# jeffreyyu0602/quantized-training

Measured on AMD Instinct MI355X. Metric: quantized_elements_per_sec, higher is better.
Workload: dtype bf16; 1 GPU; llama-2-7b-shaped LLaMA (32 layers, hidden 4096, random init) WikiText-style window eval B=1 S=1024 stride 512, fake-quant activation=e4m3 weight=e4m3, --quantize_forward gemm (weights re-quantized every forward); route=eager, parallelism=dp1 (windows round-robin, metric all_gather only), launch=hipGraph replay, valid=True

## Files before the change

### quantized-training_amd/csrc/qt_model_ops.hip

```cpp
#include <hip/hip_runtime.h>
#include <stdint.h>

#include "../../include/qt_hip.h"
#include "qt_device.h"
#include "qt_dispatch.h"
#include "qt_formats.h"
#include "qt_value_codes.h"
#include "qt_value_rows.h"

namespace {

constexpr int kNormThreads = 256;
constexpr int kNormMaxVec = 8;

struct NormExtra {
    uint2 *y8[2];
    qt_format fmt[2];
    int e5m2[2];
};

template <int FQ, bool ADD = false, int EXTRA = 0, int NV = kNormMaxVec>
__global__ __launch_bounds__(kNormThreads) void rmsnorm_kernel(const uint4 *__restrict__ x, const uint4 *__restrict__ w,
                                                               uint4 *__restrict__ y, int nvec, float inv_cols, float eps,
                                                               uint2 *__restrict__ y8, qt_format fmt,
// ... 123 lines not shown
        y[i] = uint4{o[0], o[1], o[2], o[3]};
    }
}

template <bool E5M2>
__global__ __launch_bounds__(256) void silu_mul_fq8_kernel(const uint4 *__restrict__ g, const uint4 *__restrict__ u,
                                                           uint4 *__restrict__ y, uint2 *__restrict__ y8, size_t nvec,
                                                           qt_format fmt, size_t cv, size_t rs_g, size_t rs_u) {
    for (size_t i = (size_t)blockIdx.x * 256 + threadIdx.x; i < nvec; i += (size_t)gridDim.x * 256) {
        const size_t row = i / cv, col = i - row * cv;
        const uint4 a = g[row * rs_g + col], b = u[row * rs_u + col];
        const uint32_t p[4] = {a.x, a.y, a.z, a.w}, q[4] = {b.x, b.y, b.z, b.w};
        uint32_t o[4];
#pragma unroll
        for (int j = 0; j < 4; ++j) {
            const float g0 = bf_lo(p[j]), g1 = bf_hi(p[j]);
            const float s0 = bf16_round(g0 / (1.0f + expf(-g0))), s1 = bf16_round(g1 / (1.0f + expf(-g1)));
            o[j] = pack_bf16x2(s0 * bf_lo(q[j]), s1 * bf_hi(q[j]));
        }
        const uint2 codes = fq8_hw_vec8<E5M2>(o, fmt);
        y[i] = uint4{o[0], o[1], o[2], o[3]};
        y8[i] = codes;
    }
}

struct RopeArgs {
    const uint16_t *x;
    uint16_t *y;
    const uint16_t *cos, *sin;
    long B, S, H, D;
    size_t nvec;
    long rsv;
};

__device__ __forceinline__ void rope_one(const RopeArgs &a, size_t i) {
    const long dv = a.D / 8;
    const long d8 = (long)(i % dv);
    const size_t bsh = i / dv;
    const size_t bs = bsh / (size_t)a.H;
    const long half = dv / 2;
    const bool low = d8 < half;
    const size_t in_row = bs * (size_t)a.rsv + (bsh % (size_t)a.H) * dv;
    const uint4 xv = *(const uint4 *)(a.x + (in_row + d8) * 8);
    const uint4 pv = *(const uint4 *)(a.x + (in_row + (low ? d8 + half : d8 - half)) * 8);
    const uint4 cv = *(const uint4 *)(a.cos + (bs * dv + d8) * 8);
    const uint4 sv = *(const uint4 *)(a.sin + (bs * dv + d8) * 8);
    const uint32_t X[4] = {xv.x, xv.y, xv.z, xv.w}, P[4] = {pv.x, pv.y, pv.z, pv.w};
    const uint32_t C[4] = {cv.x, cv.y, cv.z, cv.w}, S[4] = {sv.x, sv.y, sv.z, sv.w};
    const float sgn = low ? -1.0f : 1.0f;
    uint32_t o[4];
#pragma unroll
    for (int j = 0; j < 4; ++j) {
        const float a0 = bf16_round(bf_lo(X[j]) * bf_lo(C[j])), a1 = bf16_round(bf_hi(X[j]) * bf_hi(C[j]));
        const float b0 = bf16_round(sgn * bf_lo(P[j]) * bf_lo(S[j])), b1 = bf16_round(sgn * bf_hi(P[j]) * bf_hi(S[j]));
        o[j] = pack_bf16x2(a0 + b0, a1 + b1);
    }
    *(uint4 *)(a.y + i * 8) = uint4{o[0], o[1], o[2], o[3]};
}

__global__ __launch_bounds__(256) void rope_kernel(RopeArgs q, RopeArgs k) {
    const size_t total = q.nvec + k.nvec;
    for (size_t i = (size_t)blockIdx.x * 256 + threadIdx.x; i < total; i += (size_t)gridDim.x * 256) {
        if (i < q.nvec) rope_one(q, i);
        else rope_one(k, i - q.nvec);
    }
}

struct RopeFqArgs {
    RopeArgs r;
    qt_format fmt;
    uint8_t *y8;
    int e5m2;
    int inner;
    qt_format inner_fmt;
    const uint16_t *map;
    const uint16_t *rows_lds;
};

template <bool CODES = false>
__device__ __forceinline__ void rope_fq_token(const RopeFqArgs &a, size_t bs0, uint32_t tpb, size_t tokens) {
    const uint32_t dv = (uint32_t)a.r.D / 8, half = dv / 2, nv = (uint32_t)a.r.H * dv;
    const uint32_t S = (uint32_t)a.r.S;
    for (uint32_t i = threadIdx.x; i < tpb * nv; i += 256) {
        const uint32_t lt = tpb == 1 ? 0u : i / nv, v = i - lt * nv;
        const size_t bs = bs0 + lt;
        if (bs >= tokens) break;
        const uint32_t b = (uint32_t)(bs / S), s = (uint32_t)(bs - (size_t)b * S);
        const uint16_t *xrow = a.r.x + bs * (size_t)a.r.rsv * 8;
        const uint16_t *crow = a.r.cos + bs * dv * 8, *srow = a.r.sin + bs * dv * 8;
        const uint32_t h = v / dv, d8 = v - h * dv;
        const bool low = d8 < half;
        const uint4 xv = *(const uint4 *)(xrow + (size_t)v * 8);
        uint32_t out[4] = {xv.x, xv.y, xv.z, xv.w};
        if (a.r.cos) {
            const uint4 pv = *(const uint4 *)(xrow + (size_t)(low ? v + half : v - half) * 8);
            const uint4 cv = *(const uint4 *)(crow + d8 * 8);
            const uint4 sv = *(const uint4 *)(srow + d8 * 8);
            const uint32_t X[4] = {xv.x, xv.y, xv.z, xv.w}, P[4] = {pv.x, pv.y, pv.z, pv.w};
            const uint32_t C[4] = {cv.x, cv.y, cv.z, cv.w}, S[4] = {sv.x, sv.y, sv.z, sv.w};
            const float sgn = low ? -1.0f : 1.0f;
#pragma unroll
            for (int j = 0; j < 4; ++j) {
                float a0 = bf16_round(bf_lo(X[j]) * bf_lo(C[j])), a1 = bf16_round(bf_hi(X[j]) * bf_hi(C[j]));
                if (!CODES && a.inner) {
                    if (a.map) {
                        const Rounder<kFmtRows> rin{a.fmt, a.rows_lds, a.map};
                        a0 = qt_u2f(rin(qt_f2u(a0)));
                        a1 = qt_u2f(rin(qt_f2u(a1)));
                    } else {
                        a0 = qt_u2f(qt_fp_sat_u32(qt_f2u(a0), a.inner_fmt.p0, a.inner_fmt.p1, a.inner_fmt.fhi));
                        a1 = qt_u2f(qt_fp_sat_u32(qt_f2u(a1), a.inner_fmt.p0, a.inner_fmt.p1, a.inner_fmt.fhi));
                    }
                }
                const float b0 = bf16_round(sgn * bf_lo(P[j]) * bf_lo(S[j])), b1 = bf16_round(sgn * bf_hi(P[j]) * bf_hi(S[j]));
                out[j] = pack_bf16x2(a0 + b0, a1 + b1);
            }
        }
        const size_t o = (((size_t)b * (size_t)a.r.H + h) * (size_t)a.r.S + s) * dv + d8;
        if (CODES || a.y8) {
            const uint2 codes = a.e5m2 ? fq8_hw_vec8<true>(out, a.fmt) : fq8_hw_vec8<false>(out, a.fmt);
            *(uint2 *)(a.y8 + o * 8) = codes;
        } else if (a.map) {
            const Rounder<kFmtRows> rnd{a.fmt, a.rows_lds, a.map};
            const uint32_t oin[4] = {out[0], out[1], out[2], out[3]};
            fq_rows_words<4, false>(oin, out, rnd);
        } else {
#pragma unroll
            for (int j = 0; j < 4; ++j) {
                const uint32_t r0 = qt_fp_sat_u32(out[j] << 16, a.fmt.p0, a.fmt.p1, a.fmt.fhi);
                const uint32_t r1 = qt_fp_sat_u32(out[j] & 0xFFFF0000u, a.fmt.p0, a.fmt.p1, a.fmt.fhi);
                out[j] = (r0 >> 16) | (r1 & 0xFFFF0000u);
            }
        }
        if (a.r.y) *(uint4 *)(a.r.y + o * 8) = uint4{out[0], out[1], out[2], out[3]};
    }
}

__global__ __launch_bounds__(256) void rope_fq_kernel(RopeFqArgs q, RopeFqArgs k, unsigned tpb) {
    __shared__ uint4 s_rope_rows[512];
    if (q.map) {
        const uint4 *gr = (const uint4 *)(q.map + QT_MAP_ENTRIES);
        const int nrows = (q.fmt.p1 & 2) ? 512 : 256;
        for (int i = threadIdx.x; i < nrows; i += 256) s_rope_rows[i] = gr[i];
        __syncthreads();
        q.rows_lds = k.rows_lds = (const uint16_t *)s_rope_rows;
    }
    const size_t tokens = (size_t)q.r.B * (size_t)q.r.S;
    for (size_t bs = (size_t)blockIdx.x * tpb; bs < tokens; bs += (size_t)gridDim.x * tpb) {
        rope_fq_token(q, bs, tpb, tokens);
        rope_fq_token(k, bs, tpb, tokens);
    }
}

struct ValueArgs {
    const uint16_t *v;
    uint8_t *vt8;
    long sb, sh, sk, Sk;
    int H, nkb;
    qt_format fmt;
};

template <bool VE5M2, int VD, bool CODES = false>
__global__ __launch_bounds__(256) void rope_fq_value_kernel(RopeFqArgs q, RopeFqArgs k, ValueArgs v, unsigned rope_blocks, unsigned tpb) {
    __shared__ __attribute__((aligned(16))) uint8_t tile[VD * 128];
    if (blockIdx.x < rope_blocks) {
        const size_t tokens = (size_t)q.r.B * (size_t)q.r.S;
        for (size_t bs = (size_t)blockIdx.x * tpb; bs < tokens; bs += (size_t)rope_blocks * tpb) {
            rope_fq_token<CODES>(q, bs, tpb, tokens);
            rope_fq_token<CODES>(k, bs, tpb, tokens);
        }
    } else {
        const unsigned vb = blockIdx.x - rope_blocks;
        value_codes_block<VE5M2, VD>(tile, v.v, v.vt8, (int)(vb % (unsigned)v.nkb), (long)(vb / (unsigned)v.nkb), v.H, v.Sk, v.sb, v.sh, v.sk, v.fmt);
    }
}

struct ValueRowsArgs {
    const uint16_t *v;
    uint16_t *vt;
    long sb, sh, sk, Sk;
    int H, nkb;
};
struct WeightPassArgs {
    const uint4 *w;
    uint4 *wq;
    size_t nvec;
    unsigned blocks;
};

__global__ __launch_bounds__(256) void rope_map_value_kernel(RopeFqArgs q, RopeFqArgs k, ValueRowsArgs v, WeightPassArgs wp, unsigned rope_blocks,
                                                             unsigned tpb) {
    __shared__ __attribute__((aligned(16))) uint16_t tile[value_rows_tile_elems<64>()];
    __shared__ uint4 s_rows[512];
    {
        const uint4 *gr = (const uint4 *)(q.map + QT_MAP_ENTRIES);
        const int nrows = (q.fmt.p1 & 2) ? 512 : 256;
        for (int i = threadIdx.x; i < nrows; i += 256) s_rows[i] = gr[i];
        __syncthreads();
        q.rows_lds = k.rows_lds = (const uint16_t *)s_rows;
    }
    if (blockIdx.x < wp.blocks) {
        const Rounder<kFmtRows> rnd{q.fmt, (const uint16_t *)s_rows, q.map};
        constexpr int kU = 4;
        const size_t stride = (size_t)wp.blocks * 256;
        for (size_t i0 = (size_t)blockIdx.x * 256 + threadIdx.x; i0 < wp.nvec; i0 += stride * kU) {
            uint4 a[kU];
#pragma unroll
            for (int u = 0; u < kU; ++u)
                if (i0 + u * stride < wp.nvec) a[u] = wp.w[i0 + u * stride];
#pragma unroll
            for (int u = 0; u < kU; ++u) {
                if (i0 + u * stride < wp.nvec) {
                    const uint32_t in[4] = {a[u].x, a[u].y, a[u].z, a[u].w};
                    uint32_t o[4];
                    fq_rows_words<4, false>(in, o, rnd);
                    wp.wq[i0 + u * stride] = uint4{o[0], o[1], o[2], o[3]};
                }
            }
        }
        return;
    }
    const unsigned bid = blockIdx.x - wp.blocks;
    if (bid < rope_blocks) {
        const size_t tokens = (size_t)q.r.B * (size_t)q.r.S;
        for (size_t bs = (size_t)bid * tpb; bs < tokens; bs += (size_t)rope_blocks * tpb) {
            rope_fq_token(q, bs, tpb, tokens);
            rope_fq_token(k, bs, tpb, tokens);
        }
    } else {
        const unsigned vb = bid - rope_blocks;
        const Rounder<kFmtRows> rnd{q.fmt, (const uint16_t *)s_rows, q.map};
        value_t_rows_block<64>(tile, rnd, v.v, v.vt, v.H, v.Sk, v.sb, v.sh, v.sk, (long)(vb / (unsigned)v.nkb), (int)(vb % (unsigned)v.nkb), (int)threadIdx.x);
    }
}

struct LnArgs {
    const uint4 *x, *res, *w, *b;
    uint4 *y, *yq;
    uint2 *y8;
    long rows;
    int nvec;
    float inv_cols, eps;
    qt_format fmt;
    int n_extra;
    NormExtra extra;
};

template <int G, int FQ, bool ADD, int NV = kNormMaxVec>
__global__ __launch_bounds__(256) void layernorm_kernel(LnArgs a) {
    constexpr int RPB = 256 / G;
    __shared__ float s_part[2][4];
    const int sub = threadIdx.x / G, lane = threadIdx.x % G;
    const long row = (long)blockIdx.x * RPB + sub;
    if (G == 64 && row >= a.rows) return;
    const size_t base = (size_t)row * (size_t)a.nvec;
    uint4 v[NV];
    float sum = 0.0f;
#pragma unroll
    for (int i = 0; i < NV; ++i) {
        const int c = lane + i * G;
        if (c < a.nvec) {
            v[i] = a.x[base + c];
            if constexpr (ADD) {
                const uint4 r = a.res[base + c];
                v[i].x = pack_bf16x2(bf_lo(v[i].x) + bf_lo(r.x), bf_hi(v[i].x) + bf_hi(r.x));
                v[i].y = pack_bf16x2(bf_lo(v[i].y) + bf_lo(r.y), bf_hi(v[i].y) + bf_hi(r.y));
                v[i].z = pack_bf16x2(bf_lo(v[i].z) + bf_lo(r.z), bf_hi(v[i].z) + bf_hi(r.z));
                v[i].w = pack_bf16x2(bf_lo(v[i].w) + bf_lo(r.w), bf_hi(v[i].w) + bf_hi(r.w));
            }
            sum += (bf_lo(v[i].x) + bf_hi(v[i].x)) + (bf_lo(v[i].y) + bf_hi(v[i].y)) + (bf_lo(v[i].z) + bf_hi(v[i].z)) +
                   (bf_lo(v[i].w) + bf_hi(v[i].w));
        }
    }
    auto reduce = [&](float t, int slot) {
#pragma unroll
        for (int off = 32; off >= 1; off >>= 1) t += __shfl_xor(t, off, 64);
        if constexpr (G == 256) {
            if ((threadIdx.x & 63) == 0) s_part[slot][threadIdx.x >> 6] = t;
            __syncthreads();
            t = (s_part[slot][0] + s_part[slot][1]) + (s_part[slot][2] + s_part[slot][3]);
        }
        return t;
    };
    const float mean = reduce(sum, 0) * a.inv_cols;
    float sq = 0.0f;
#pragma unroll
    for (int i = 0; i < NV; ++i) {
        const int c = lane + i * G;
        if (c < a.nvec) {
            const uint32_t q[4] = {v[i].x, v[i].y, v[i].z, v[i].w};
#pragma unroll
            for (int j = 0; j < 4; ++j) {
                const float d0 = bf_lo(q[j]) - mean, d1 = bf_hi(q[j]) - mean;
                sq += d0 * d0;
                sq += d1 * d1;
            }
        }
    }
    const float rstd = rsqrtf(reduce(sq, 1) * a.inv_cols + a.eps);
#pragma unroll
    for (int i = 0; i < NV; ++i) {
        const int c = lane + i * G;
        if (c < a.nvec) {
            const uint4 ww = a.w[c], bb = a.b[c];
            const uint32_t q[4] = {v[i].x, v[i].y, v[i].z, v[i].w}, g[4] = {ww.x, ww.y, ww.z, ww.w}, h[4] = {bb.x, bb.y, bb.z, bb.w};
            uint32_t o[4];
#pragma unroll
            for (int j = 0; j < 4; ++j)
                o[j] = pack_bf16x2(bf_lo(g[j]) * (rstd * (bf_lo(q[j]) - mean)) + bf_lo(h[j]),
                                   bf_hi(g[j]) * (rstd * (bf_hi(q[j]) - mean)) + bf_hi(h[j]));
            a.y[base + c] = uint4{o[0], o[1], o[2], o[3]};
            if constexpr (FQ != 0) {
                for (int e = 0; e < a.n_extra; ++e) {
                    uint32_t t[4] = {o[0], o[1], o[2], o[3]};
                    a.extra.y8[e][base + c] = a.extra.e5m2[e] ? fq8_hw_vec8<true>(t, a.extra.fmt[e]) : fq8_hw_vec8<false>(t, a.extra.fmt[e]);
                }
                const uint2 codes = fq8_hw_vec8<FQ == 2>(o, a.fmt);
                if (a.yq) a.yq[base + c] = uint4{o[0], o[1], o[2], o[3]};
                a.y8[base + c] = codes;
            }
        }
    }
// ... 263 lines not shown
static int launch_layernorm_any(const LnArgs &a, int fq, bool with_residual, void *stream);

int qt_layernorm_bf16(const uint16_t *x, const uint16_t *residual, const uint16_t *weight, const uint16_t *bias, uint16_t *y,
                      uint16_t *yq, uint8_t *y8, long rows, long cols, float eps, const qt_format *fmt, void *stream) {
    if (rows * cols == 0) return QT_OK;
    if (!x || !weight || !bias || !y || rows < 0 || cols < 0 || (yq && !y8)) return QT_ERR_BAD_ARG;
    const int fq = y8 ? qt_fp8_code(fmt) : 0;
    if (y8 && !fq) return QT_ERR_BAD_ARG;
    if (cols % 8 || cols > (long)kNormThreads * kNormMaxVec * 8 ||
        (((uintptr_t)x | (uintptr_t)residual | (uintptr_t)weight | (uintptr_t)bias | (uintptr_t)y | (uintptr_t)yq) & 15u) || ((uintptr_t)y8 & 7u))
        return QT_ERR_UNALIGNED;
    LnArgs a{(const uint4 *)x, (const uint4 *)residual, (const uint4 *)weight, (const uint4 *)bias, (uint4 *)y, (uint4 *)yq, (uint2 *)y8,
             rows, (int)(cols / 8), 1.0f / (float)cols, eps, fmt && fq ? *fmt : qt_format{}, 0, NormExtra{}};
    return launch_layernorm_any(a, fq, residual != nullptr, stream);
}

int qt_layernorm_consumers_bf16(const uint16_t *x, const uint16_t *residual, const uint16_t *weight, const uint16_t *bias, uint16_t *y,
                                uint16_t *yq, long rows, long cols, float eps, int consumers, uint8_t *const *y8,
                                const qt_format *const *fmt, void *stream) {
    if (rows * cols == 0) return QT_OK;
    if (!x || !weight || !bias || !y || rows < 0 || cols < 0 || consumers < 2 || consumers > 3 || !y8 || !fmt) return QT_ERR_BAD_ARG;
    int code[3] = {0, 0, 0};
    for (int i = 0; i < consumers; ++i) {
        if (!y8[i] || !fmt[i] || ((uintptr_t)y8[i] & 7u)) return QT_ERR_BAD_ARG;
        code[i] = qt_fp8_code(fmt[i]);
        if (!code[i]) return QT_ERR_BAD_ARG;
    }
    if (cols % 8 || cols > (long)kNormThreads * kNormMaxVec * 8 ||
        (((uintptr_t)x | (uintptr_t)residual | (uintptr_t)weight | (uintptr_t)bias | (uintptr_t)y | (uintptr_t)yq) & 15u))
        return QT_ERR_UNALIGNED;
    LnArgs a{(const uint4 *)x, (const uint4 *)residual, (const uint4 *)weight, (const uint4 *)bias, (uint4 *)y, (uint4 *)yq, (uint2 *)y8[0],
             rows, (int)(cols / 8), 1.0f / (float)cols, eps, *fmt[0], consumers - 1, NormExtra{}};
    for (int i = 1; i < consumers; ++i) {
        a.extra.y8[i - 1] = (uint2 *)y8[i];
        a.extra.fmt[i - 1] = *fmt[i];
        a.extra.e5m2[i - 1] = code[i] == 2;
    }
    return launch_layernorm_any(a, code[0], residual != nullptr, stream);
}

static int launch_layernorm_any(const LnArgs &a, int fq, bool with_residual, void *stream) {
    hipStream_t st = (hipStream_t)stream;
    const long rows = a.rows;
    const bool residual = with_residual;
    if (a.nvec <= 128) {
        const unsigned blocks = (unsigned)((rows + 3) / 4);
        if (residual) launch_layernorm<64, true>(a, fq, blocks, st);
        else launch_layernorm<64, false>(a, fq, blocks, st);
    } else {
        if (residual) launch_layernorm<256, true>(a, fq, (unsigned)rows, st);
        else launch_layernorm<256, false>(a, fq, (unsigned)rows, st);
    }
    return qt_launch_status();
}

int qt_gelu_bf16(const uint16_t *x, uint16_t *y, uint8_t *y8, size_t n, const qt_format *fmt, void *stream) {
    if (n == 0) return QT_OK;
    if (!x || (!y && !y8)) return QT_ERR_BAD_ARG;
    const int fq = y8 ? qt_fp8_code(fmt) : 0;
    if (y8 && !fq) return QT_ERR_BAD_ARG;
    if ((n & 7) || (((uintptr_t)x | (uintptr_t)y) & 15u) || ((uintptr_t)y8 & 7u)) return QT_ERR_UNALIGNED;
    const size_t nvec = n / 8;
    size_t blocks = (nvec + 255) / 256;
    if (blocks > 256 * 32) blocks = 256 * 32;
    hipStream_t st = (hipStream_t)stream;
    const qt_format f = fq ? *fmt : qt_format{};
    qt_pick<0, 1, 2>(fq, [&](auto FQ) {
        gelu_kernel<decltype(FQ)::value><<<(unsigned)blocks, 256, 0, st>>>((const uint4 *)x, (uint4 *)y, (uint2 *)y8, nvec, f);
    });
    return qt_launch_status();
}

int qt_silu_mul_bf16(const uint16_t *gate, const uint16_t *up, uint16_t *y, size_t rows, size_t cols, size_t gate_row_stride,
                     size_t up_row_stride, void *stream) {
    const size_t n = rows * cols;
    if (n == 0) return QT_OK;
    if (!gate || !up || !y || gate_row_stride < cols || up_row_stride < cols) return QT_ERR_BAD_ARG;
    if ((cols & 7) || ((gate_row_stride | up_row_stride) & 7) || (((uintptr_t)gate | (uintptr_t)up | (uintptr_t)y) & 15u))
        return QT_ERR_UNALIGNED;
    const size_t nvec = n / 8;
    size_t blocks = (nvec + 255) / 256;
    if (blocks > 256 * 32) blocks = 256 * 32;
    silu_mul_kernel<<<(unsigned)blocks, 256, 0, (hipStream_t)stream>>>((const uint4 *)gate, (const uint4 *)up, (uint4 *)y, nvec,
                                                                       cols / 8, gate_row_stride / 8, up_row_stride / 8);
    return qt_launch_status();
}

int qt_silu_mul_fq8_bf16(const uint16_t *gate, const uint16_t *up, uint16_t *y, uint8_t *y8, size_t rows, size_t cols,
                         size_t gate_row_stride, size_t up_row_stride, const qt_format *fmt, void *stream) {
    const size_t n = rows * cols;
    if (n == 0) return QT_OK;
    const int f8 = qt_fp8_code(fmt);
    if (!gate || !up || !y || !y8 || !f8 || gate_row_stride < cols || up_row_stride < cols) return QT_ERR_BAD_ARG;
    if ((cols & 7) || ((gate_row_stride | up_row_stride) & 7) || (((uintptr_t)gate | (uintptr_t)up | (uintptr_t)y) & 15u) ||
        ((uintptr_t)y8 & 7u))
        return QT_ERR_UNALIGNED;
    const size_t nvec = n / 8;
    size_t blocks = (nvec + 255) / 256;
    if (blocks > 256 * 32) blocks = 256 * 32;
    qt_pick_bool(f8 == 2, [&](auto E5M2) {
        silu_mul_fq8_kernel<decltype(E5M2)::value><<<(unsigned)blocks, 256, 0, (hipStream_t)stream>>>((const uint4 *)gate, (const uint4 *)up, (uint4 *)y, (uint2 *)y8, nvec,
                                                                                                      *fmt, cols / 8, gate_row_stride / 8, up_row_stride / 8);
    });
    return qt_launch_status();
}

int qt_rope_bf16(const uint16_t *q, const uint16_t *k, const uint16_t *cos, const uint16_t *sin, uint16_t *q_out,
                 uint16_t *k_out, long B, long S, long Hq, long Hk, long D, long q_row_stride, long k_row_stride, void *stream) {
    if (B * S * D == 0) return QT_OK;
    if (!q || !k || !cos || !sin || !q_out || !k_out || B < 0 || S < 0 || Hq < 0 || Hk < 0) return QT_ERR_BAD_ARG;
    if (D % 16 || (((uintptr_t)q | (uintptr_t)k | (uintptr_t)cos | (uintptr_t)sin | (uintptr_t)q_out | (uintptr_t)k_out) & 15u))
        return QT_ERR_UNALIGNED;
    if (q_row_stride < Hq * D || k_row_stride < Hk * D || (q_row_stride | k_row_stride) % 8) return QT_ERR_BAD_ARG;
    RopeArgs aq{q, q_out, cos, sin, B, S, Hq, D, (size_t)(B * S * Hq * D / 8), q_row_stride / 8};
    RopeArgs ak{k, k_out, cos, sin, B, S, Hk, D, (size_t)(B * S * Hk * D / 8), k_row_stride / 8};
    size_t blocks = (aq.nvec + ak.nvec + 255) / 256;
    if (blocks > 256 * 32) blocks = 256 * 32;
    rope_kernel<<<(unsigned)blocks, 256, 0, (hipStream_t)stream>>>(aq, ak);
    return qt_launch_status();
}

static int rope_fq_launch(const uint16_t *q, const uint16_t *k, const uint16_t *cos, const uint16_t *sin, uint16_t *q_out, uint16_t *k_out,
                          uint8_t *q_out8, uint8_t *k_out8, long B, long S, long Hq, long Hk, long D, long q_row_stride, long k_row_stride,
                          const qt_format *fmt_q, const qt_format *fmt_k, bool need_values, const uint16_t *v, uint8_t *vt8, long v_sb, long v_sh,
                          long v_sk, const qt_format *fmt_v, void *stream, const qt_format *inner_q = nullptr, const qt_format *inner_k = nullptr) {
    if (B * S * D == 0) return QT_OK;
    if ((inner_q && inner_q->kind != QT_FMT_FP_SAT) || (inner_k && inner_k->kind != QT_FMT_FP_SAT) || ((inner_q || inner_k) && !cos)) return QT_ERR_BAD_ARG;
    if (!q || !k || (need_values && !cos) || (cos == nullptr) != (sin == nullptr) || !fmt_q || !fmt_k || B < 0 || S < 0 || Hq < 0 || Hk < 0)
        return QT_ERR_BAD_ARG;
    if (need_values ? (!q_out || !k_out) : (!q_out8 || !k_out8 || (q_out == nullptr) != (k_out == nullptr))) return QT_ERR_BAD_ARG;
    if (fmt_q->kind != QT_FMT_FP_SAT || fmt_k->kind != QT_FMT_FP_SAT) return QT_ERR_BAD_ARG;
    if (D % 16 || (((uintptr_t)q | (uintptr_t)k | (uintptr_t)cos | (uintptr_t)sin | (uintptr_t)q_out | (uintptr_t)k_out) & 15u))
        return QT_ERR_UNALIGNED;
    if (q_row_stride < Hq * D || k_row_stride < Hk * D || (q_row_stride | k_row_stride) % 8) return QT_ERR_BAD_ARG;
    if (((uintptr_t)q_out8 | (uintptr_t)k_out8) & 7u) return QT_ERR_UNALIGNED;
    if ((q_out8 && !qt_fp8_code(fmt_q)) || (k_out8 && !qt_fp8_code(fmt_k))) return QT_ERR_BAD_ARG;
    RopeFqArgs aq{{q, q_out, cos, sin, B, S, Hq, D, (size_t)(B * S * Hq * D / 8), q_row_stride / 8}, *fmt_q, q_out8, qt_fp8_code(fmt_q) == 2 ? 1 : 0,
                  inner_q ? 1 : 0, inner_q ? *inner_q : qt_format{}, nullptr, nullptr};
    RopeFqArgs ak{{k, k_out, cos, sin, B, S, Hk, D, (size_t)(B * S * Hk * D / 8), k_row_stride / 8}, *fmt_k, k_out8, qt_fp8_code(fmt_k) == 2 ? 1 : 0,
                  inner_k ? 1 : 0, inner_k ? *inner_k : qt_format{}, nullptr, nullptr};
    if (Hq * D / 8 > 0xFFFFFFFFl || Hk * D / 8 > 0xFFFFFFFFl || B > 0x7FFFFFFFl || S > 0x7FFFFFFFl) return QT_ERR_BAD_ARG;
    const long nv_max = (Hq > Hk ? Hq : Hk) * D / 8;
    const unsigned tpb = nv_max >= 256 || nv_max < 1 ? 1u : (unsigned)(256 / nv_max);
    size_t blocks = ((size_t)B * (size_t)S + tpb - 1) / tpb;
    if (blocks > 256 * 64) blocks = 256 * 64;
    hipStream_t st = (hipStream_t)stream;
    if (!v) {
        rope_fq_kernel<<<(unsigned)blocks, 256, 0, st>>>(aq, ak, tpb);
        return qt_launch_status();
    }
    if (!vt8 || !qt_fp8_code(fmt_v) || (D != 64 && D != 128) || S % 128 != 0 || B * Hk > 65535) return QT_ERR_BAD_ARG;
    if ((((uintptr_t)v | (uintptr_t)vt8) & 15u) || ((v_sb | v_sh | v_sk) & 7)) return QT_ERR_UNALIGNED;
    ValueArgs av{v, vt8, v_sb, v_sh, v_sk, S, (int)Hk, (int)(S / 128), *fmt_v};
    const unsigned total = (unsigned)blocks + (unsigned)(B * Hk * (S / 128));
    const bool ve5 = qt_fp8_code(fmt_v) == 2;
    if (D == 128) {
        const bool codes = aq.y8 && ak.y8 && !aq.inner && !ak.inner && !aq.map && !ak.map;
        if (codes && !ve5) rope_fq_value_kernel<false, 128, true><<<total, 256, 0, st>>>(aq, ak, av, (unsigned)blocks, tpb);
        else if (ve5) rope_fq_value_kernel<true, 128><<<total, 256, 0, st>>>(aq, ak, av, (unsigned)blocks, tpb);
        else rope_fq_value_kernel<false, 128><<<total, 256, 0, st>>>(aq, ak, av, (unsigned)blocks, tpb);
    } else {
        const bool codes = aq.y8 && ak.y8 && !aq.inner && !ak.inner && !aq.map && !ak.map;
        if (codes && !ve5) rope_fq_value_kernel<false, 64, true><<<total, 256, 0, st>>>(aq, ak, av, (unsigned)blocks, tpb);
        else if (ve5) rope_fq_value_kernel<true, 64><<<total, 256, 0, st>>>(aq, ak, av, (unsigned)blocks, tpb);
        else rope_fq_value_kernel<false, 64><<<total, 256, 0, st>>>(aq, ak, av, (unsigned)blocks, tpb);
    }
    return qt_launch_status();
}

int qt_rope_fq_bf16(const uint16_t *q, const uint16_t *k, const uint16_t *cos, const uint16_t *sin, uint16_t *q_out,
                    uint16_t *k_out, uint8_t *q_out8, uint8_t *k_out8, long B, long S, long Hq, long Hk, long D,
                    long q_row_stride, long k_row_stride, const qt_format *fmt_q, const qt_format *fmt_k, void *stream) {
    return rope_fq_launch(q, k, cos, sin, q_out, k_out, q_out8, k_out8, B, S, Hq, Hk, D, q_row_stride, k_row_stride, fmt_q, fmt_k, true, nullptr,
                          nullptr, 0, 0, 0, nullptr, stream);
}

int qt_rope_fq_value(const uint16_t *q, const uint16_t *k, const uint16_t *cos, const uint16_t *sin, uint16_t *q_out, uint16_t *k_out,
                     uint8_t *q_out8, uint8_t *k_out8, long B, long S, long Hq, long Hk, long D, long q_row_stride, long k_row_stride,
                     const qt_format *fmt_q, const qt_format *fmt_k, const uint16_t *v, uint8_t *vt8, long v_stride_b, long v_stride_h,
                     long v_stride_k, const qt_format *fmt_v, void *stream) {
    return rope_fq_launch(q, k, cos, sin, q_out, k_out, q_out8, k_out8, B, S, Hq, Hk, D, q_row_stride, k_row_stride, fmt_q, fmt_k, false, v, vt8,
                          v_stride_b, v_stride_h, v_stride_k, fmt_v, stream);
}

static bool map_format_ok(const qt_format *fmt, const uint16_t *map) {
    return fmt && map && fmt->kind == QT_FMT_LUT && (fmt->p1 & 1) && (((uintptr_t)map) & 15u) == 0;
}

int qt_rmsnorm_map_bf16(const uint16_t *x, const uint16_t *residual, const uint16_t *weight, uint16_t *sum, uint16_t *y, long rows, long cols,
                        float eps, const qt_format *fmt, const uint16_t *map, int quantize_sum, void *stream) {
    if (rows * cols == 0) return QT_OK;
    if (!x || !weight || !y || rows < 0 || cols < 0 || (residual != nullptr) != (sum != nullptr) || !map_format_ok(fmt, map)) return QT_ERR_BAD_ARG;
    if (cols % 8 || cols > (long)kNormThreads * kNormMaxVec * 8 ||
        (((uintptr_t)x | (uintptr_t)residual | (uintptr_t)weight | (uintptr_t)sum | (uintptr_t)y) & 15u))
        return QT_ERR_UNALIGNED;
    hipStream_t st = (hipStream_t)stream;
    const int nvec = (int)(cols / 8);
    const float inv = 1.0f / (float)cols;
    if (residual) launch_rms<3, true, 0>((unsigned)rows, nvec, st, (const uint4 *)x, (const uint4 *)weight, (uint4 *)y, nvec, inv, eps, nullptr, *fmt, (const uint4 *)residual, (uint4 *)sum, NormExtra{}, quantize_sum ? 3 : 0, qt_format{}, map);
    else launch_rms<3, false, 0>((unsigned)rows, nvec, st, (const uint4 *)x, (const uint4 *)weight, (uint4 *)y, nvec, inv, eps, nullptr, *fmt, nullptr, nullptr, NormExtra{}, 0, qt_format{}, map);
    return qt_launch_status();
}

int qt_silu_mul_map_bf16(const uint16_t *gate, const uint16_t *up, uint16_t *y, size_t rows, size_t cols, size_t gate_row_stride,
                         size_t up_row_stride, const qt_format *fmt, const uint16_t *map, void *stream) {
    if (rows * cols == 0) return QT_OK;
    if (!gate || !up || !y || !map_format_ok(fmt, map)) return QT_ERR_BAD_ARG;
    if (cols % 8 || gate_row_stride % 8 || up_row_stride % 8 || gate_row_stride < cols || up_row_stride < cols ||
        (((uintptr_t)gate | (uintptr_t)up | (uintptr_t)y) & 15u))
        return QT_ERR_UNALIGNED;
    const size_t nvec = rows * cols / 8;
    size_t blocks = (nvec + 255) / 256;
    if (blocks > 256 * 32) blocks = 256 * 32;
    silu_mul_map_kernel<<<(unsigned)blocks, 256, 0, (hipStream_t)stream>>>((const uint4 *)gate, (const uint4 *)up, (uint4 *)y, nvec, *fmt, map, cols / 8,
                                                                          gate_row_stride / 8, up_row_stride / 8);
    return qt_launch_status();
}

int qt_rope_map_bf16(const uint16_t *q, const uint16_t *k, const uint16_t *cos, const uint16_t *sin, uint16_t *q_out, uint16_t *k_out, long B,
                     long S, long Hq, long Hk, long D, long q_row_stride, long k_row_stride, const qt_format *fmt, const uint16_t *map,
                     int inner_q, int inner_k, void *stream) {
    if (B * S * D == 0) return QT_OK;
    if (!q || !k || !cos || !sin || !q_out || !k_out || B < 0 || S < 0 || Hq < 0 || Hk < 0 || !map_format_ok(fmt, map)) return QT_ERR_BAD_ARG;
    if (D % 16 || (((uintptr_t)q | (uintptr_t)k | (uintptr_t)cos | (uintptr_t)sin | (uintptr_t)q_out | (uintptr_t)k_out) & 15u))
        return QT_ERR_UNALIGNED;
    if (q_row_stride < Hq * D || k_row_stride < Hk * D || (q_row_stride | k_row_stride) % 8) return QT_ERR_BAD_ARG;
    if (Hq * D / 8 > 0xFFFFFFFFl || Hk * D / 8 > 0xFFFFFFFFl || B > 0x7FFFFFFFl || S > 0x7FFFFFFFl) return QT_ERR_BAD_ARG;
    RopeFqArgs aq{{q, q_out, cos, sin, B, S, Hq, D, (size_t)(B * S * Hq * D / 8), q_row_stride / 8}, *fmt, nullptr, 0, inner_q ? 1 : 0, qt_format{}, map, nullptr};
    RopeFqArgs ak{{k, k_out, cos, sin, B, S, Hk, D, (size_t)(B * S * Hk * D / 8), k_row_stride / 8}, *fmt, nullptr, 0, inner_k ? 1 : 0, qt_format{}, map, nullptr};
    const long nv_max = (Hq > Hk ? Hq : Hk) * D / 8;
    const unsigned tpb = nv_max >= 256 || nv_max < 1 ? 1u : (unsigned)(256 / nv_max);
    size_t blocks = ((size_t)B * (size_t)S + tpb - 1) / tpb;
    if (blocks > 256 * 64) blocks = 256 * 64;
    rope_fq_kernel<<<(unsigned)blocks, 256, 0, (hipStream_t)stream>>>(aq, ak, tpb);
    return qt_launch_status();
}

static int rope_map_value_launch(const uint16_t *q, const uint16_t *k, const uint16_t *cos, const uint16_t *sin, uint16_t *q_out, uint16_t *k_out,
                                 long B, long S, long Hq, long Hk, long D, long q_row_stride, long k_row_stride, const qt_format *fmt,
                                 const uint16_t *map, int inner_q, int inner_k, const uint16_t *v, uint16_t *vt, long v_stride_b, long v_stride_h,
                                 long v_stride_k, const uint16_t *w, uint16_t *wq, size_t w_elems, void *stream) {
    if (B * S * D == 0) return QT_OK;
    if (!q || !k || !cos || !sin || !q_out || !k_out || !v || !vt || B < 0 || S < 0 || Hq < 0 || Hk < 1 || !map_format_ok(fmt, map)) return QT_ERR_BAD_ARG;
    if (D != kValueRowsD || S % 128 != 0 || B * Hk > 65535 || (w_elems != 0 && (!w || !wq))) return QT_ERR_BAD_ARG;
    if ((((uintptr_t)q | (uintptr_t)k | (uintptr_t)cos | (uintptr_t)sin | (uintptr_t)q_out | (uintptr_t)k_out | (uintptr_t)v | (uintptr_t)vt) & 15u) ||
        ((v_stride_b | v_stride_h | v_stride_k) & 7) || (w_elems != 0 && ((((uintptr_t)w | (uintptr_t)wq) & 15u) || (w_elems & 7))))
        return QT_ERR_UNALIGNED;
    if (q_row_stride < Hq * D || k_row_stride < Hk * D || (q_row_stride | k_row_stride) % 8) return QT_ERR_BAD_ARG;
    if (Hq * D / 8 > 0xFFFFFFFFl || Hk * D / 8 > 0xFFFFFFFFl || B > 0x7FFFFFFFl || S > 0x7FFFFFFFl) return QT_ERR_BAD_ARG;
    RopeFqArgs aq{{q, q_out, cos, sin, B, S, Hq, D, (size_t)(B * S * Hq * D / 8), q_row_stride / 8}, *fmt, nullptr, 0, inner_q ? 1 : 0, qt_format{}, map, nullptr};
    RopeFqArgs ak{{k, k_out, cos, sin, B, S, Hk, D, (size_t)(B * S * Hk * D / 8), k_row_stride / 8}, *fmt, nullptr, 0, inner_k ? 1 : 0, qt_format{}, map, nullptr};
    const long nv_max = (Hq > Hk ? Hq : Hk) * D / 8;
    const unsigned tpb = nv_max >= 256 || nv_max < 1 ? 1u : (unsigned)(256 / nv_max);
    size_t blocks = ((size_t)B * (size_t)S + tpb - 1) / tpb;
    if (blocks > 256 * 64) blocks = 256 * 64;
    ValueRowsArgs av{v, vt, v_stride_b, v_stride_h, v_stride_k, S, (int)Hk, (int)(S / 64)};
    WeightPassArgs aw{(const uint4 *)w, (uint4 *)wq, w_elems / 8, 0};
    if (aw.nvec) {
        size_t wb = (aw.nvec + 256 * 4 - 1) / (256 * 4);
        if (wb > 256 * 2) wb = 256 * 2;
        aw.blocks = (unsigned)wb;
    }
    const unsigned total = aw.blocks + (unsigned)blocks + (unsigned)(B * Hk * (S / 64));
    rope_map_value_kernel<<<total, 256, 0, (hipStream_t)stream>>>(aq, ak, av, aw, (unsigned)blocks, tpb);
    return qt_launch_status();
}

int qt_rope_map_value(const uint16_t *q, const uint16_t *k, const uint16_t *cos, const uint16_t *sin, uint16_t *q_out, uint16_t *k_out, long B,
                      long S, long Hq, long Hk, long D, long q_row_stride, long k_row_stride, const qt_format *fmt, const uint16_t *map,
                      int inner_q, int inner_k, const uint16_t *v, uint16_t *vt, long v_stride_b, long v_stride_h, long v_stride_k, void *stream) {
    return rope_map_value_launch(q, k, cos, sin, q_out, k_out, B, S, Hq, Hk, D, q_row_stride, k_row_stride, fmt, map, inner_q, inner_k, v, vt,
                                 v_stride_b, v_stride_h, v_stride_k, nullptr, nullptr, 0, stream);
}

int qt_rope_map_value_weight(const uint16_t *q, const uint16_t *k, const uint16_t *cos, const uint16_t *sin, uint16_t *q_out, uint16_t *k_out, long B,
                             long S, long Hq, long Hk, long D, long q_row_stride, long k_row_stride, const qt_format *fmt, const uint16_t *map,
                             int inner_q, int inner_k, const uint16_t *v, uint16_t *vt, long v_stride_b, long v_stride_h, long v_stride_k,
                             const uint16_t *w, uint16_t *wq, size_t w_elems, void *stream) {
    return rope_map_value_launch(q, k, cos, sin, q_out, k_out, B, S, Hq, Hk, D, q_row_stride, k_row_stride, fmt, map, inner_q, inner_k, v, vt,
                                 v_stride_b, v_stride_h, v_stride_k, w, wq, w_elems, stream);
}

int qt_rope_fq_inner_value(const uint16_t *q, const uint16_t *k, const uint16_t *cos, const uint16_t *sin, uint16_t *q_out, uint16_t *k_out,
                           uint8_t *q_out8, uint8_t *k_out8, long B, long S, long Hq, long Hk, long D, long q_row_stride, long k_row_stride,
                           const qt_format *fmt_q, const qt_format *fmt_k, const qt_format *inner_q, const qt_format *inner_k, const uint16_t *v,
                           uint8_t *vt8, long v_stride_b, long v_stride_h, long v_stride_k, const qt_format *fmt_v, void *stream) {
    return rope_fq_launch(q, k, cos, sin, q_out, k_out, q_out8, k_out8, B, S, Hq, Hk, D, q_row_stride, k_row_stride, fmt_q, fmt_k, false, v, vt8,
                          v_stride_b, v_stride_h, v_stride_k, fmt_v, stream, inner_q, inner_k);
}

int qt_causal_lm_loss_bf16(const uint16_t *logits, const long long *labels, long batch, long seq_len, long vocab, long row_stride,
                           long long ignore_index, float *row_loss_scratch, float *loss_out, void *stream) {
    if (!logits || !labels || !row_loss_scratch || !loss_out || batch < 1 || seq_len < 1 || vocab < 1 || row_stride < vocab) return QT_ERR_BAD_ARG;
    if (((uintptr_t)logits & 15u) || (row_stride & 7)) return QT_ERR_UNALIGNED;
    const long rows = batch * seq_len;
    if (rows > 0x7FFFFFFFl) return QT_ERR_BAD_ARG;
    hipStream_t st = (hipStream_t)stream;
    nll_rows_kernel<<<(unsigned)rows, 256, 0, st>>>(logits, labels, seq_len, vocab, row_stride, ignore_index, row_loss_scratch);
    nll_mean_kernel<<<1, 256, 0, st>>>(row_loss_scratch, rows, loss_out);
    return qt_launch_status();
}

int qt_colsum_bf16(const uint16_t *x_dev, uint16_t *out_dev, long rows, long cols, void *stream) {
    if (rows < 0 || cols < 0) return QT_ERR_BAD_ARG;
    if (cols == 0) return QT_OK;
    if (!x_dev || !out_dev || cols % 8 != 0) return QT_ERR_BAD_ARG;
    if ((uintptr_t)x_dev & 15u) return QT_ERR_UNALIGNED;
    colsum_kernel<<<(unsigned)((cols + 31) / 32), 256, 0, (hipStream_t)stream>>>(x_dev, out_dev, rows, cols);
    return qt_launch_status();
}

}
```

### quantized-training_amd/csrc/qt_value_codes.h

```cpp
#pragma once
#include "qt_device.h"

namespace {

template <bool E5M2, int D>
__device__ __forceinline__ void value_codes_block(uint8_t *tile , const uint16_t *v, uint8_t *vt8, int kb, long bh, int H,
                                                  long Sk, long sb, long sh, long sk, const qt_format &fmt) {
    const int t = threadIdx.x;
    const long b = bh / H, h = bh % H;
#pragma unroll
    for (int it = 0; it < D / 16; ++it) {
        const int vi = it * 256 + t, key = vi / (D / 8), dv = vi % (D / 8);
        const uint4 in = *(const uint4 *)(v + b * sb + h * sh + ((long)kb * 128 + key) * sk + dv * 8);
        uint32_t o[4] = {in.x, in.y, in.z, in.w};
        const uint2 codes = fq8_hw_vec8<E5M2>(o, fmt);
        const int p = (key & 64) | (((key >> 2) & 3) << 4) | (((key >> 4) & 3) << 2) | (key & 3);
#pragma unroll
        for (int j = 0; j < 8; ++j) tile[(dv * 8 + j) * 128 + p] = (uint8_t)((j < 4 ? codes.x >> (8 * j) : codes.y >> (8 * (j - 4))) & 0xFFu);
    }
    __syncthreads();
#pragma unroll
    for (int it = 0; it < D / 32; ++it) {
        const int ci = it * 256 + t, d = ci >> 3, ch = ci & 7;
        *(uint4 *)(vt8 + (bh * D + d) * Sk + (long)kb * 128 + ch * 16) = *(const uint4 *)(tile + d * 128 + ch * 16);
    }
}

}
```

Baseline: 890.4 billion elements/s.

## Fuse Q/K rope into one-pass fp8 codes and transpose V codes via shuffles

Adds a one-pass RoPE path that loads the Q and K halves together, rotates them and emits fp8 codes with vectorised 16-byte stores, using a fast code path with a rare fallback for special values. It also rewrites the V transpose so that byte-granular LDS scatter stores are replaced by in-wave lane shuffles and XOR-swizzled 16-byte LDS writes. The aim is to cut LDS byte stores, bank conflicts and per-token overhead in the fused rope/value kernel. It adds complexity in the lane-exchange logic and changes the threads-per-block mapping for rope blocks.

```diff
diff --git a/quantized-training_amd/csrc/qt_model_ops.hip b/quantized-training_amd/csrc/qt_model_ops.hip
--- a/quantized-training_amd/csrc/qt_model_ops.hip
+++ b/quantized-training_amd/csrc/qt_model_ops.hip
@@ -299,6 +299,64 @@
     }
 }
 
+template <bool E5M2, int D>
+__device__ __forceinline__ void rope_codes_one_pass(const RopeFqArgs &q, const RopeFqArgs &k, size_t bs0, uint32_t tpb, size_t tokens) {
+    constexpr uint32_t C = D / 32, dv = D / 8;
+    const uint32_t Hq = (uint32_t)q.r.H, Hk = (uint32_t)k.r.H, P = (Hq > Hk ? Hq : Hk) * C;
+    const uint32_t i = threadIdx.x;
+    if (i >= tpb * P) return;
+    const uint32_t lt = tpb == 1 ? 0u : i / P, j = i - lt * P;
+    const size_t bs = bs0 + lt;
+    if (bs >= tokens) return;
+    const uint32_t S = (uint32_t)q.r.S, b = (uint32_t)(bs / S), s = (uint32_t)(bs - (size_t)b * S);
+    const uint32_t h = j / C, c = j % C;
+    const bool rot = q.r.cos != nullptr, doq = h < Hq, dok = h < Hk;
+    const uint4 z = uint4{0u, 0u, 0u, 0u};
+    uint4 xq[4] = {z, z, z, z}, xk[4] = {z, z, z, z}, cs[4] = {z, z, z, z}, sn[4] = {z, z, z, z};
+    const size_t head = (size_t)h * D + 16 * c;
+    if (doq) {
+        const uint4 *x = (const uint4 *)(q.r.x + bs * (size_t)q.r.rsv * 8 + head);
+        xq[0] = x[0], xq[1] = x[1], xq[2] = x[dv / 2], xq[3] = x[dv / 2 + 1];
+    }
+    if (dok) {
+        const uint4 *x = (const uint4 *)(k.r.x + bs * (size_t)k.r.rsv * 8 + head);
+        xk[0] = x[0], xk[1] = x[1], xk[2] = x[dv / 2], xk[3] = x[dv / 2 + 1];
+    }
+    if (rot) {
+        const uint4 *cr = (const uint4 *)(q.r.cos + bs * D + 16 * c), *sr = (const uint4 *)(q.r.sin + bs * D + 16 * c);
+        cs[0] = cr[0], cs[1] = cr[1], cs[2] = cr[dv / 2], cs[3] = cr[dv / 2 + 1];
+        sn[0] = sr[0], sn[1] = sr[1], sn[2] = sr[dv / 2], sn[3] = sr[dv / 2 + 1];
+    }
+    float neg = -1.0f;
+    asm volatile("" : "+v"(neg));
+    auto side = [&](const RopeFqArgs &a, const uint4 (&x)[4]) {
+        uint32_t out[4][4];
+#pragma unroll
+        for (int u = 0; u < 4; ++u) {
+            const uint4 pv = x[u ^ 2];
+            const uint32_t X[4] = {x[u].x, x[u].y, x[u].z, x[u].w}, Pw[4] = {pv.x, pv.y, pv.z, pv.w};
+            const uint32_t Cw[4] = {cs[u].x, cs[u].y, cs[u].z, cs[u].w}, Sw[4] = {sn[u].x, sn[u].y, sn[u].z, sn[u].w};
+#pragma unroll
+            for (int w = 0; w < 4; ++w) {
+                out[u][w] = X[w];
+                if (rot) {
+                    const float a0 = bf16_round(bf_lo(X[w]) * bf_lo(Cw[w])), a1 = bf16_round(bf_hi(X[w]) * bf_hi(Cw[w]));
+                    const float p0 = u < 2 ? neg * bf_lo(Pw[w]) : bf_lo(Pw[w]), p1 = u < 2 ? neg * bf_hi(Pw[w]) : bf_hi(Pw[w]);
+                    const float b0 = bf16_round(p0 * bf_lo(Sw[w])), b1 = bf16_round(p1 * bf_hi(Sw[w]));
+                    out[u][w] = pack_bf16x2(a0 + b0, a1 + b1);
+                }
+            }
+        }
+        uint2 codes[4];
+        fq8_codes_vecs<E5M2, 4>(out, codes, a.fmt);
+        const size_t o = (((size_t)b * (size_t)a.r.H + h) * (size_t)a.r.S + s) * D + 16 * c;
+        *(uint4 *)(a.y8 + o) = uint4{codes[0].x, codes[0].y, codes[1].x, codes[1].y};
+        *(uint4 *)(a.y8 + o + D / 2) = uint4{codes[2].x, codes[2].y, codes[3].x, codes[3].y};
+    };
+    if (doq) side(q, xq);
+    if (dok) side(k, xk);
+}
+
 struct ValueArgs {
     const uint16_t *v;
     uint8_t *vt8;
@@ -307,14 +365,19 @@
     qt_format fmt;
 };
 
-template <bool VE5M2, int VD, bool CODES = false>
+template <bool VE5M2, int VD, bool CODES = false, int ONE = 0>
 __global__ __launch_bounds__(256) void rope_fq_value_kernel(RopeFqArgs q, RopeFqArgs k, ValueArgs v, unsigned rope_blocks, unsigned tpb) {
+    static_assert(ONE == 0 || (CODES && !VE5M2), "the one-pass path is the codes-only mode's");
     __shared__ __attribute__((aligned(16))) uint8_t tile[VD * 128];
     if (blockIdx.x < rope_blocks) {
         const size_t tokens = (size_t)q.r.B * (size_t)q.r.S;
         for (size_t bs = (size_t)blockIdx.x * tpb; bs < tokens; bs += (size_t)rope_blocks * tpb) {
-            rope_fq_token<CODES>(q, bs, tpb, tokens);
-            rope_fq_token<CODES>(k, bs, tpb, tokens);
+            if constexpr (ONE != 0) {
+                rope_codes_one_pass<ONE == 2, VD>(q, k, bs, tpb, tokens);
+            } else {
+                rope_fq_token<CODES>(q, bs, tpb, tokens);
+                rope_fq_token<CODES>(k, bs, tpb, tokens);
+            }
         }
     } else {
         const unsigned vb = blockIdx.x - rope_blocks;
@@ -884,19 +947,28 @@
     if (!vt8 || !qt_fp8_code(fmt_v) || (D != 64 && D != 128) || S % 128 != 0 || B * Hk > 65535) return QT_ERR_BAD_ARG;
     if ((((uintptr_t)v | (uintptr_t)vt8) & 15u) || ((v_sb | v_sh | v_sk) & 7)) return QT_ERR_UNALIGNED;
     ValueArgs av{v, vt8, v_sb, v_sh, v_sk, S, (int)Hk, (int)(S / 128), *fmt_v};
+    const bool ve5 = qt_fp8_code(fmt_v) == 2;
+    const bool codes = aq.y8 && ak.y8 && !aq.inner && !ak.inner && !aq.map && !ak.map;
+    const long pairs = (Hq > Hk ? Hq : Hk) * (D / 32);
+    const bool one = codes && !ve5 && D % 32 == 0 && aq.e5m2 == ak.e5m2 && pairs >= 1 && pairs <= 256 &&
+                     !(((uintptr_t)q_out8 | (uintptr_t)k_out8) & 15u);
+    unsigned tpb_l = tpb;
+    if (one) {
+        tpb_l = (unsigned)(256 / pairs);
+        blocks = ((size_t)B * (size_t)S + tpb_l - 1) / tpb_l;
+        if (blocks > 256 * 64) blocks = 256 * 64;
+    }
     const unsigned total = (unsigned)blocks + (unsigned)(B * Hk * (S / 128));
-    const bool ve5 = qt_fp8_code(fmt_v) == 2;
-    if (D == 128) {
-        const bool codes = aq.y8 && ak.y8 && !aq.inner && !ak.inner && !aq.map && !ak.map;
-        if (codes && !ve5) rope_fq_value_kernel<false, 128, true><<<total, 256, 0, st>>>(aq, ak, av, (unsigned)blocks, tpb);
-        else if (ve5) rope_fq_value_kernel<true, 128><<<total, 256, 0, st>>>(aq, ak, av, (unsigned)blocks, tpb);
-        else rope_fq_value_kernel<false, 128><<<total, 256, 0, st>>>(aq, ak, av, (unsigned)blocks, tpb);
-    } else {
-        const bool codes = aq.y8 && ak.y8 && !aq.inner && !ak.inner && !aq.map && !ak.map;
-        if (codes && !ve5) rope_fq_value_kernel<false, 64, true><<<total, 256, 0, st>>>(aq, ak, av, (unsigned)blocks, tpb);
-        else if (ve5) rope_fq_value_kernel<true, 64><<<total, 256, 0, st>>>(aq, ak, av, (unsigned)blocks, tpb);
-        else rope_fq_value_kernel<false, 64><<<total, 256, 0, st>>>(aq, ak, av, (unsigned)blocks, tpb);
-    }
+    const int route = one ? 3 + aq.e5m2 : ve5 ? 2 : codes ? 1 : 0;
+    qt_pick_bool(D == 128, [&](auto D128) {
+        constexpr int VD = decltype(D128)::value ? 128 : 64;
+        qt_pick<0, 1, 2, 3, 4>(route, [&](auto R) {
+            constexpr int r = decltype(R)::value;
+            constexpr int kOne = r < 3 ? 0 : r - 2;
+            constexpr bool kCodes = r == 1 || kOne != 0;
+            rope_fq_value_kernel<r == 2, VD, kCodes, kOne><<<total, 256, 0, st>>>(aq, ak, av, (unsigned)blocks, tpb_l);
+        });
+    });
     return qt_launch_status();
 }
 
diff --git a/quantized-training_amd/csrc/qt_value_codes.h b/quantized-training_amd/csrc/qt_value_codes.h
--- a/quantized-training_amd/csrc/qt_value_codes.h
+++ b/quantized-training_amd/csrc/qt_value_codes.h
@@ -3,26 +3,92 @@
 
 namespace {
 
+template <bool E5M2, int N>
+__device__ __forceinline__ void fq8_codes_vecs(uint32_t (&w)[N][4], uint2 (&codes)[N], const qt_format &fmt) {
+    uint32_t special = 0;
+#pragma unroll
+    for (int n = 0; n < N; ++n) {
+        const uint32_t m = pk_max_u16(pk_max_u16(w[n][0] & 0x7FFF7FFFu, w[n][1] & 0x7FFF7FFFu), pk_max_u16(w[n][2] & 0x7FFF7FFFu, w[n][3] & 0x7FFF7FFFu));
+        special |= ((((m & 0xFFFFu) >= 0x7F80u) | ((m >> 16) >= 0x7F80u)) ? 1u : 0u) << n;
+        codes[n] = uint2{fq8_fast_word4<E5M2>(w[n][0], w[n][1]), fq8_fast_word4<E5M2>(w[n][2], w[n][3])};
+    }
+    if (__builtin_expect(special != 0, 0)) {
+#pragma clang loop unroll(disable)
+        for (int n = 0; n < N; ++n) {
+            if (special & 1u) {
+                float f[8];
+#pragma unroll
+                for (int j = 0; j < 4; ++j) {
+                    f[2 * j] = qt_u2f(qt_fp_sat_u32(w[0][j] << 16, fmt.p0, fmt.p1, fmt.fhi));
+                    f[2 * j + 1] = qt_u2f(qt_fp_sat_u32(w[0][j] & 0xFFFF0000u, fmt.p0, fmt.p1, fmt.fhi));
+                }
+                codes[0] = uint2{qt_pack_fp8x4<E5M2>(f[0], f[1], f[2], f[3]), qt_pack_fp8x4<E5M2>(f[4], f[5], f[6], f[7])};
+            }
+            special >>= 1;
+            const uint32_t w0[4] = {w[0][0], w[0][1], w[0][2], w[0][3]};
+            const uint2 c0 = codes[0];
+#pragma unroll
+            for (int k = 0; k + 1 < N; ++k) {
+#pragma unroll
+                for (int j = 0; j < 4; ++j) w[k][j] = w[k + 1][j];
+                codes[k] = codes[k + 1];
+            }
+#pragma unroll
+            for (int j = 0; j < 4; ++j) w[N - 1][j] = w0[j];
+            codes[N - 1] = c0;
+        }
+    }
+}
+
 template <bool E5M2, int D>
 __device__ __forceinline__ void value_codes_block(uint8_t *tile , const uint16_t *v, uint8_t *vt8, int kb, long bh, int H,
                                                   long Sk, long sb, long sh, long sk, const qt_format &fmt) {
-    const int t = threadIdx.x;
+    static_assert(D == 64 || D == 128, "lanes D / 8 and D / 4 apart exchange inside one wavefront");
+    constexpr int DV = D / 8;
+    constexpr int GL = 16 / DV;
+    constexpr int GW = 4 / GL;
+    constexpr int QW = 4 / GW;
+    constexpr int NQ = 2 / QW;
+    const int t = threadIdx.x, lane = t & 63, wave = t >> 6;
     const long b = bh / H, h = bh % H;
+    const int dv = lane % DV, e = (lane / DV) & 3, g = (wave % GW) * GL + lane / (4 * DV);
+    const uint16_t *vb = v + b * sb + h * sh + (long)kb * 128 * sk + dv * 8;
+    uint32_t w[NQ * 4][4];
 #pragma unroll
-    for (int it = 0; it < D / 16; ++it) {
-        const int vi = it * 256 + t, key = vi / (D / 8), dv = vi % (D / 8);
-        const uint4 in = *(const uint4 *)(v + b * sb + h * sh + ((long)kb * 128 + key) * sk + dv * 8);
-        uint32_t o[4] = {in.x, in.y, in.z, in.w};
-        const uint2 codes = fq8_hw_vec8<E5M2>(o, fmt);
-        const int p = (key & 64) | (((key >> 2) & 3) << 4) | (((key >> 4) & 3) << 2) | (key & 3);
+    for (int qi = 0; qi < NQ; ++qi)
 #pragma unroll
-        for (int j = 0; j < 8; ++j) tile[(dv * 8 + j) * 128 + p] = (uint8_t)((j < 4 ? codes.x >> (8 * j) : codes.y >> (8 * (j - 4))) & 0xFFu);
+        for (int tt = 0; tt < 4; ++tt) {
+            const int key = 64 * (qi * QW + wave / GW) + 16 * tt + 4 * g + e;
+            const uint4 in = *(const uint4 *)(vb + (long)key * sk);
+            w[qi * 4 + tt][0] = in.x, w[qi * 4 + tt][1] = in.y, w[qi * 4 + tt][2] = in.z, w[qi * 4 + tt][3] = in.w;
+        }
+    uint2 cd[NQ * 4];
+    fq8_codes_vecs<E5M2, NQ * 4>(w, cd, fmt);
+    const bool e1 = e & 2, e0 = e & 1;
+#pragma unroll
+    for (int qi = 0; qi < NQ; ++qi) {
+        uint32_t rx[4], ry[4];
+#pragma unroll
+        for (int tt = 0; tt < 4; ++tt) {
+            const uint2 codes = cd[qi * 4 + tt];
+            const uint32_t s1 = e1 ? ((codes.x & 0xFFFFu) | (codes.y << 16)) : ((codes.x >> 16) | (codes.y & 0xFFFF0000u));
+            const uint32_t r1 = (uint32_t)__shfl_xor((int)s1, 2 * DV, 64);
+            const uint32_t x1 = e1 ? ((r1 & 0xFFFFu) | (codes.x & 0xFFFF0000u)) : ((codes.x & 0xFFFFu) | (r1 << 16));
+            const uint32_t y1 = e1 ? ((r1 >> 16) | (codes.y & 0xFFFF0000u)) : ((codes.y & 0xFFFFu) | (r1 & 0xFFFF0000u));
+            const uint32_t s2 = e0 ? ((x1 & 0x00FF00FFu) | ((y1 << 8) & 0xFF00FF00u)) : (((x1 >> 8) & 0x00FF00FFu) | (y1 & 0xFF00FF00u));
+            const uint32_t r2 = (uint32_t)__shfl_xor((int)s2, DV, 64);
+            rx[tt] = e0 ? ((r2 & 0x00FF00FFu) | (x1 & 0xFF00FF00u)) : ((x1 & 0x00FF00FFu) | ((r2 & 0x00FF00FFu) << 8));
+            ry[tt] = e0 ? (((r2 >> 8) & 0x00FF00FFu) | (y1 & 0xFF00FF00u)) : ((y1 & 0x00FF00FFu) | (r2 & 0xFF00FF00u));
+        }
+        const int piece = (4 * (qi * QW + wave / GW) + g) ^ (dv & 7);
+        *(uint4 *)(tile + (dv * 8 + e) * 128 + piece * 16) = uint4{rx[0], rx[1], rx[2], rx[3]};
+        *(uint4 *)(tile + (dv * 8 + 4 + e) * 128 + piece * 16) = uint4{ry[0], ry[1], ry[2], ry[3]};
     }
     __syncthreads();
 #pragma unroll
     for (int it = 0; it < D / 32; ++it) {
         const int ci = it * 256 + t, d = ci >> 3, ch = ci & 7;
-        *(uint4 *)(vt8 + (bh * D + d) * Sk + (long)kb * 128 + ch * 16) = *(const uint4 *)(tile + d * 128 + ch * 16);
+        *(uint4 *)(vt8 + (bh * D + d) * Sk + (long)kb * 128 + ch * 16) = *(const uint4 *)(tile + d * 128 + ((ch ^ ((d >> 3) & 7)) * 16));
     }
 }
 
```

Result: no change. 888.6 billion elements/s (-0.2%).
